# IamJerryXu/Multimodal-Diagnosis-HAM-Spine

Hardware: AMD Instinct MI355X
Metric: training images/sec, ResNet50+BERT-base 224px bs32 (higher is better)
Workload: dtype bf16; 1 GPU; C2: ResNet50 + BERT-base(L=128) + cross-attention FusionModule + MLP head, 224x224, batch 32 per GPU, CE(label_smoothing=0.02), fused AdamW, train-mode BatchNorm and dropout; per_gpu_batch=32, global_batch=32, seq_len=128, params=134897991, parallelism=dp1

## Files before the change

include/hamspine.h:

```cpp
#ifndef HAMSPINE_H
#define HAMSPINE_H

#include <stdint.h>

#ifdef __cplusplus
extern "C" {
#endif

typedef int hs_status;
enum { HS_OK = 0, HS_ERR_ARG = 1, HS_ERR_HIP = 2, HS_ERR_UNSUPPORTED = 3 };
enum { HS_F32 = 0, HS_BF16 = 1 };

const char* hs_last_error(void);
int hs_version(void);
int hs_device_ok(void);


enum {
    HS_A_KC = 0,
    HS_A_RC = 1,
    HS_A_CONV = 2,
    HS_A_DGRAD = 3
};
enum {
// ... 381 lines not shown
                            int32_t order, float grid_eps, float one_minus_eps, float margin, void* ws, int64_t ws_bytes,
                            void* stream);
int64_t hs_kan_refit_ws_bytes(int64_t B, int32_t in_f, int32_t out_f, int32_t grid_size, int32_t order, int32_t y_mode);
hs_status hs_kan_refit(const float* x, const float* grid_new, const float* grid_old, const float* y, const float* spline_w,
                       const float* scaler, float* out, int64_t B, int32_t in_f, int32_t out_f, int32_t grid_size, int32_t order,
                       void* ws, int64_t ws_bytes, void* stream);
hs_status hs_moe_gate_fwd(const float* clean, const float* raw_noise, const float* noise, int32_t B, int32_t E, int32_t k, int32_t noisy,
                          float noise_eps, uint64_t seed, float coef, float* gates, float* p, int32_t* top, float* z,
                          float* sigma, float* loadrow, float* loss, float* d_imp, float* d_load, void* stream);
hs_status hs_moe_gate_bwd(const float* clean, const float* raw_noise, const float* p, const int32_t* top, const float* z,
                          const float* sigma, const float* dgates, const float* g_loss, const float* d_imp,
                          const float* d_load, int32_t B, int32_t E, int32_t k, int32_t noisy, float* d_clean, float* d_raw,
                          void* stream);
hs_status hs_moe_combine_fwd(const float* gates, const float* const* outs, float* y, int32_t B, int32_t E, int32_t O,
                             void* stream);
hs_status hs_moe_combine_bwd(const float* gates, const float* const* outs, const float* dy, float* const* douts,
                             float* dgates, int32_t B, int32_t E, int32_t O, void* stream);

int32_t hs_pointwise_stat_rows(int64_t M, int32_t N, int32_t K);
hs_status hs_pointwise_fwd(const void* x, int64_t M, int32_t K, int32_t ldx, const void* w, int32_t N, void* y, int32_t ldy,
                           float* stats, void* stream);

hs_status hs_moe_dispatch_index(const float* gates, int32_t B, int32_t E, int32_t* idx, int32_t* count, void* stream);
hs_status hs_rows_gather(const float* src, const int32_t* idx, float* dst, int32_t n, int32_t D, void* stream);
hs_status hs_rows_scatter_add(float* dst, const int32_t* idx, const float* scale, int32_t ld_scale, int32_t col, const float* src,
                              int32_t n, int32_t D, void* stream);
hs_status hs_rows_scatter_add_bwd(const float* dy, const int32_t* idx, const float* gates, int32_t E, int32_t col, const float* src,
                                  float* dsrc, float* dgates, int32_t n, int32_t D, void* stream);


typedef struct hs_attn_desc {
    int32_t dtype;
    int32_t B, H, Lq, Lk, hd;
    int64_t q_bs, k_bs, v_bs, o_bs;
    int32_t q_ld, k_ld, v_ld, o_ld;
    float scale;
    float dropout_p;
    uint64_t seed;
    const int64_t* key_mask;
} hs_attn_desc;
hs_status hs_attention_query(const hs_attn_desc* d, int64_t* saved_bytes, int64_t* ws_bytes);
hs_status hs_attention_fwd(const hs_attn_desc* d, const void* q, const void* k, const void* v, void* o, void* saved,
                           int64_t saved_bytes, void* ws, int64_t ws_bytes, void* stream);
hs_status hs_attention_bwd(const hs_attn_desc* d, const void* q, const void* k, const void* v, const void* d_o, void* dq,
                           void* dk, void* dv, void* saved, int64_t saved_bytes, void* ws, int64_t ws_bytes,
                           void* stream);

void hs_set_overlap(int32_t on);
hs_status hs_grad_milestones(int32_t n, const void* const* grad_ptrs, void* const* events);
int32_t hs_measure_build(void);
void hs_set_wgrad_nt(int32_t on);
void hs_set_bert_wgrad_chunks(int32_t on);
void hs_set_pack_xcd_spread(int32_t on);
int64_t hs_gemm_k_cols_queued(void);

typedef struct hs_conv_bn {
    int32_t Cin, Cout, R, stride, pad;
    const float* w;
    const float* gamma;
    const float* beta;
    float* running_mean;
    float* running_var;
    float* dw;
    float* dgamma;
    float* dbeta;
} hs_conv_bn;

typedef struct hs_resblock_desc {
    int32_t dtype;
    int32_t N, H, W;
    int32_t training;
    float eps, momentum;
    int32_t n_main;
    hs_conv_bn main[3];
    int32_t has_ds;
    hs_conv_bn ds;
    int32_t inference;
} hs_resblock_desc;
hs_status hs_resblock_query(const hs_resblock_desc* d, int64_t* saved_bytes, int64_t* ws_bytes);
hs_status hs_resblock_fwd(const hs_resblock_desc* d, const void* x, void* y, void* saved, int64_t saved_bytes, void* ws,
                          int64_t ws_bytes, void* stream);
hs_status hs_resblock_bwd(const hs_resblock_desc* d, const void* x, const void* y, const void* dy, void* dx, void* saved,
                          int64_t saved_bytes, void* ws, int64_t ws_bytes, void* stream);

typedef struct hs_stem_desc {
    int32_t dtype;
    int32_t N, H, W;
    int32_t training;
    float eps, momentum;
    hs_conv_bn cb;
    int32_t inference;
} hs_stem_desc;
hs_status hs_stem_query(const hs_stem_desc* d, int64_t* saved_bytes, int64_t* ws_bytes);
hs_status hs_stem_fwd(const hs_stem_desc* d, const float* image, void* y, void* saved, int64_t saved_bytes, void* ws,
                      int64_t ws_bytes, void* stream);
hs_status hs_stem_bwd(const hs_stem_desc* d, const void* y, const void* dy, void* saved, int64_t saved_bytes, void* ws,
                      int64_t ws_bytes, void* stream);

typedef struct hs_linear {
    int32_t in_f, out_f;
    const float* w;
    const float* b;
    float* dw;
    float* db;
} hs_linear;
typedef struct hs_norm {
// ... 147 lines not shown
```

multimodal-diagnosis-ham-spine_amd/hamspine/csrc/gemm.hip:

```cpp
#include <atomic>
#include <mutex>
#include <unordered_set>
#include <vector>
#include <stdarg.h>
#include <math.h>
#include <map>
#include <tuple>
#include "gemm_launch.h"
#include "gemm_p8.h"
#include "hs_internal.h"
#include "hs_switch.h"

namespace hs {

static thread_local char g_err[512] = "";
void set_error(const char* fmt, ...) {
    va_list ap;
    va_start(ap, fmt);
    vsnprintf(g_err, sizeof(g_err), fmt, ap);
    va_end(ap);
}
const char* last_error() { return g_err; }

bool lds_attr_needed(const void* fn) {
// ... 22 lines not shown
        r.a = g_prof_pool.back().first;
        r.b = g_prof_pool.back().second;
        g_prof_pool.pop_back();
    } else if (hipEventCreate(&r.a) != hipSuccess || hipEventCreate(&r.b) != hipSuccess) {
        return false;
    }
    r.flops = flops;
    r.cls = cls;
    (void)hipEventRecord(r.a, s);
    return true;
}
static void prof_end(hipStream_t s, ProfRec& r) {
    (void)hipEventRecord(r.b, s);
    std::lock_guard<std::mutex> lk(g_prof_mu);
    g_prof.push_back(r);
}

__global__ void null_kernel() {}

static constexpr int kTicketPool = 16384;
static unsigned* ticket_pool(hipStream_t s) {
    static std::mutex mu;
    static std::map<std::pair<int, hipStream_t>, unsigned*> pools;
    int dev = 0;
    if (hipGetDevice(&dev) != hipSuccess) return nullptr;
    std::lock_guard<std::mutex> lk(mu);
    auto it = pools.find({dev, s});
    if (it != pools.end()) return it->second;
    unsigned* p = nullptr;
    if (hipMalloc(&p, kTicketPool * sizeof(unsigned)) != hipSuccess) return nullptr;
    if (hipMemsetAsync(p, 0, kTicketPool * sizeof(unsigned), s) != hipSuccess) return nullptr;
    pools[{dev, s}] = p;
    return p;
}

static int g_dbg_cfg = -1, g_dbg_ablate = 0;
static unsigned long long* g_dbg_stamps = nullptr;

static int combo_of(int ak, int bk) {
    if (ak == HS_A_KC && bk == HS_B_KC) return 0;
    if (ak == HS_A_KC && bk == HS_B_RC) return 1;
    if (ak == HS_A_RC && bk == HS_B_RC) return 2;
    if (ak == HS_A_CONV && bk == HS_B_KC) return 3;
    if (ak == HS_A_DGRAD && bk == HS_B_WDGRAD) return 4;
    if (ak == HS_A_RC && bk == HS_B_CONV) return 5;
    return -1;
}

static bool aligned16(const void* p) { return (((uintptr_t)p) & 15) == 0; }

static bool batch_is_one(const hs_gemm_params* p) { return p->batch <= 1; }
static int p8_cfg(const hs_gemm_params* p) {
    if (p->M % 256 == 0 && p->N % 256 == 0 && (long long)(p->M / 256) * (p->N / 256) >= 128) return CFG_P8_256;
    return -1;
}
static int auto_cfg(const hs_gemm_params* p, bool vec) {
    const long long z = (long long)(p->batch > 0 ? p->batch : 1) * (p->split_k > 1 ? p->split_k : 1);
    const long long t12864 = (long long)ceil_div(p->M, 128) * ceil_div(p->N, 64) * z;
    const long long t128 = (long long)ceil_div(p->M, 128) * ceil_div(p->N, 128) * z;
    if (p->dtype == HS_BF16) {
        const bool plain = (p->a_kind == HS_A_KC || p->a_kind == HS_A_RC) && (p->b_kind == HS_B_KC || p->b_kind == HS_B_RC);
        if (plain && batch_is_one(p)) {
            if (p->a_kind == HS_A_KC && p->split_k <= 1 && p->N >= 2048 && p->K <= 1024 && p->M >= 2048 && p->K % 32 == 0) return CFG_128x128x32;
            if (p->a_kind == HS_A_KC && p->b_kind == HS_B_KC && p->split_k <= 1 && p->K >= 2048 && t12864 >= 256) return CFG_128x64;
        }
        return t12864 >= 1536 ? CFG_128x64 : CFG_64x64;
    }
    return (vec && t128 >= 200) ? CFG_128x128 : CFG_64x64;
}
static bool conv3_plan(const hs_gemm_params* p, int* rows, int* tpi, int* fm) {
    if (!sw::conv3() || g_dbg_cfg >= 0) return false;
    const hs_conv_geom& g = p->g;
    if (p->dtype != HS_BF16 || p->a_kind != HS_A_CONV || p->b_kind != HS_B_KC || p->split_k > 1 || p->batch > 1) return false;
    if (g.R != 3 || g.S != 3 || g.stride != 1 || g.pad != 1 || g.P != g.H || g.Q != g.W || g.C % 64 != 0 || p->N % 64 != 0) return false;
    if (g.row_pitch != g.W * g.C || g.img_pitch != g.H * g.W * g.C || g.qstep != g.C || g.no_bounds) return false;
    if (p->bias || p->colscale || p->act != HS_ACT_NONE || p->residual || p->D_preact || p->mul_mode != HS_MUL_NONE || p->dropout_p > 0.f ||
        p->accumulate || p->seg_rows > 0 || p->alpha != 1.f || p->out_dtype != HS_BF16 || p->rowsum_a || p->bnb_partials)
        return false;
    if (p->ldd % 8 != 0 || (((uintptr_t)p->D) & 15) != 0 || p->ldb != 9 * g.C || p->K != 9 * g.C || p->N != g.K) return false;
    if (g.W > 112 || g.W < 1) return false;
    const int rmax = std::min(g.H, 112 / g.W);
    const int t = ceil_div(g.H, rmax), r = ceil_div(g.H, t);
    const int tp = r * g.W;
    if (tp < 32 || (r + 2) * (g.W + 2) > 256) return false;
    *rows = r;
    *tpi = t;
    *fm = tp > 64 ? 7 : 4;
    return true;
}
int gemm_stat_rows(const hs_gemm_params* p) {
    if (!p || p->dtype != HS_BF16 || p->split_k > 1 || p->batch > 1) return 0;
    {
        int r, t, fm;
        if (conv3_plan(p, &r, &t, &fm)) return p->g.N * t;
    }
    int cfg = (p->a_kind == HS_A_CONV && p->b_kind == HS_B_KC && p->g.C % 64 != 0) ? CFG_STEM : auto_cfg(p, true);
    if (g_dbg_cfg >= 0 && g_dbg_cfg <= CFG_64x64 && cfg != CFG_STEM) cfg = g_dbg_cfg;
    if (g_dbg_cfg >= CFG_256x128 && g_dbg_cfg <= CFG_256x128x32 && !(p->a_kind == HS_A_CONV || p->a_kind == HS_A_DGRAD || p->b_kind == HS_B_CONV)) cfg = g_dbg_cfg;
    return ceil_div(p->M, cfg == CFG_64x64 ? 64 : (cfg == CFG_256x128 || cfg == CFG_256x128x32) ? 256 : 128);
}

static bool bn_finish_variant(int cfg, int combo) {
    return (combo == 0 && (cfg == CFG_64x64 || cfg == CFG_128x64)) || (combo == 3 && (cfg == CFG_64x64 || cfg == CFG_128x64 || cfg == CFG_STEM || cfg == CFG_C3));
}

struct Prepared {
// ... 540 lines not shown
    if (g_group_immediate_hook) HS_PROPAGATE(g_group_immediate_hook(g_group_immediate_ctx));
    return gemm_impl(p, s);
}
bool gemm_group_takes_k_cols() { return g_dbg_cfg < 0 && !g_dbg_stamps; }
static std::atomic<long long> g_k_cols_queued{0};
int gemm_group_add(GemmGroup* g, const hs_gemm_params* p, hipStream_t s, const int* k_cols) {
    HS_REQUIRE(!k_cols || (g && p && p->a_kind == HS_A_KC && p->b_kind == HS_B_KC), "gemm_group_add: k_cols needs an open group and K-contiguous operands");
    if (!g) return launch_ungrouped(p, s);
    Prepared q;
    const bool big = p->a_kind == HS_A_KC && p->b_kind == HS_B_KC;
    const bool p8w = sw::p8_wgrad();
    const bool want_p8 = big && p8w && p->dtype == HS_BF16 && p->M % 256 == 0 && p->N % 256 == 0 && p->K % 64 == 0 && p->K >= 2048 &&
                         (p->batch <= 1) && p->split_k <= 1 && g_dbg_cfg < 0 && (g->items.empty() || g->combo != 0 || g->cfg == CFG_P8_256);
    HS_PROPAGATE(gemm_prepare(p, s, q, big ? (want_p8 ? CFG_P8_256 : CFG_256x128) : -1));
    if (want_p8 && !(p8_epilogue_supported(q.a) && !q.a.colstats && !q.a.bnb_partials && (long long)p->M * p->lda * 2 < 0x7fffff00ll &&
                     (long long)p->N * p->ldb * 2 < 0x7fffff00ll))
        HS_PROPAGATE(gemm_prepare(p, s, q, CFG_256x128));
    const bool ok = big ? (q.bf16 && (q.cfg == CFG_256x128 || q.cfg == CFG_P8_256) && q.combo == 0 && q.batch == 1 && q.split == 1 && !q.a.stamps && !q.a.colstats)
                        : (q.bf16 && q.cfg == CFG_64x64 && (q.combo == 2 || q.combo == 5) && q.batch == 1 && !q.a.stamps &&
                           (q.split == 1 || q.a.tickets != nullptr) && !q.a.colstats &&
                           (!q.a.rowsum[0] || (q.combo == 2 && q.split == 1)));
    HS_REQUIRE(!k_cols || ok, "gemm_group_add: a problem with chunk-compacted K columns cannot be queued (gemm_group_takes_k_cols)");
    if (!ok) return launch_ungrouped(p, s);
    const long long ngroups = q.split > 1 ? (q.split + kSplitGroup - 1) / kSplitGroup : 0;
    const long long need = q.split > 1 ? (long long)q.a.tiles_m * q.a.tiles_n * (1 + (ngroups > 1 ? ngroups : 0)) : 0;
    if (!g->items.empty() && (g->combo != q.combo || (big && g->cfg != q.cfg) || (int)g->items.size() >= kGroupMax || g->ticket_off + need > kTicketPool)) {
        if (g_group_immediate_hook) HS_PROPAGATE(g_group_immediate_hook(g_group_immediate_ctx));
        HS_PROPAGATE(gemm_group_flush(g, s));
    }
    if (need > kTicketPool) return launch_ungrouped(p, s);
    q.a.k_cols = k_cols;
    if (k_cols) g_k_cols_queued.fetch_add(1, std::memory_order_relaxed);
    g->combo = q.combo;
    if (big) {
        g->cfg = q.cfg;
        g->rs = g->rs || q.a.rowsum[0] != nullptr;
    }
    if (q.split > 1) q.a.tickets += g->ticket_off;
    g->ticket_off += (int)need;
    g->first.push_back(g->total);
    g->total += (int)(q.grid.x * q.grid.z);
    g->items.push_back(q.a);
    g->flops += q.flops;
    const double R2 = q.conv ? (double)p->g.R * p->g.S : 1.0, st2 = q.conv ? (double)p->g.stride * p->g.stride : 1.0;
    g->bytes += 2.0 * ((double)p->M * p->K + (double)p->N * p->K / R2 * st2) + 4.0 * (double)p->M * p->N;
    return HS_OK;
}

}

extern "C" {
void hs_gemm_debug_stamps(void* device_buffer) { hs::g_dbg_stamps = (unsigned long long*)device_buffer; }
void hs_set_pack_xcd_spread(int32_t on) { hs::sw::set_pack_xcd_spread(on); }
int64_t hs_gemm_k_cols_queued(void) { return hs::g_k_cols_queued.load(std::memory_order_relaxed); }
void hs_gemm_debug(int32_t cfg_override, int32_t ablate) {
    hs::g_dbg_cfg = cfg_override;
    hs::g_dbg_ablate = ablate;
}
void hs_prof_enable(int32_t on) {
    std::lock_guard<std::mutex> lk(hs::g_prof_mu);
    hs::g_prof_on = on != 0;
}
hs_status hs_prof_collect(double* flops, double* ms, int64_t* launches) {
    HS_CHECK_HIP(hipDeviceSynchronize());
    std::lock_guard<std::mutex> lk(hs::g_prof_mu);
    for (int i = 0; i < 4; ++i) {
        flops[i] = 0;
        ms[i] = 0;
        launches[i] = 0;
    }
    for (auto& r : hs::g_prof) {
        float t = 0.f;
        if (hipEventElapsedTime(&t, r.a, r.b) == hipSuccess) {
            flops[r.cls] += r.flops;
            ms[r.cls] += t;
            launches[r.cls] += 1;
        }
        hs::g_prof_pool.emplace_back(r.a, r.b);
    }
    hs::g_prof.clear();
    return HS_OK;
}
hs_status hs_prof_calibrate(void* stream, int32_t n, float* avg_us) {
    HS_REQUIRE(n > 0 && avg_us, "hs_prof_calibrate: bad argument");
    hipStream_t s = (hipStream_t)stream;
    std::vector<std::pair<hipEvent_t, hipEvent_t>> ev(n);
    for (auto& e : ev) {
        HS_CHECK_HIP(hipEventCreate(&e.first));
        HS_CHECK_HIP(hipEventCreate(&e.second));
    }
    for (auto& e : ev) {
        HS_CHECK_HIP(hipEventRecord(e.first, s));
        hipLaunchKernelGGL(hs::null_kernel, dim3(1), dim3(64), 0, s);
        HS_CHECK_HIP(hipEventRecord(e.second, s));
    }
    HS_CHECK_HIP(hipStreamSynchronize(s));
    double tot = 0;
    for (auto& e : ev) {
        float t = 0.f;
        HS_CHECK_HIP(hipEventElapsedTime(&t, e.first, e.second));
        tot += t;
        (void)hipEventDestroy(e.first);
        (void)hipEventDestroy(e.second);
    }
    *avg_us = (float)(tot / n * 1e3);
    return HS_OK;
// ... 50 lines not shown
```

multimodal-diagnosis-ham-spine_amd/hamspine/csrc/gemm_bf16_p8.hip:

```cpp
#include "gemm_launch.h"
#include "gemm_p8.h"
namespace hs {
__global__ __launch_bounds__(512) void gemm_bf16_p8_256_diag_kernel(const GemmArgs a) {
    gemm_bf16_p8_body<256, 256, 2, 4, false, true, true>(a, blockIdx.x);
}
template <typename K>
static int launch_p8(K kernel, int lds, int threads, const GemmArgs& a, dim3 grid, hipStream_t s) {
    if (lds_attr_needed((const void*)kernel)) HS_CHECK_HIP(hipFuncSetAttribute((const void*)kernel, hipFuncAttributeMaxDynamicSharedMemorySize, lds));
    hipLaunchKernelGGL(kernel, grid, dim3(threads), lds, s, a);
    HS_LAUNCH_CHECK();
    return HS_OK;
}
int launch_bf16_p8_grouped(const GemmArgs* list, const int* first_wg, int n, int total_wgs, bool rs, hipStream_t s) {
    constexpr int lds = 128 * 1024;
    if (rs) {
        auto kernel = gemm_bf16_p8_grouped_kernel<true>;
        if (lds_attr_needed((const void*)kernel)) HS_CHECK_HIP(hipFuncSetAttribute((const void*)kernel, hipFuncAttributeMaxDynamicSharedMemorySize, lds));
        hipLaunchKernelGGL(kernel, dim3(total_wgs), dim3(512), lds, s, list, first_wg, n);
    } else {
        auto kernel = gemm_bf16_p8_grouped_kernel<false>;
        if (lds_attr_needed((const void*)kernel)) HS_CHECK_HIP(hipFuncSetAttribute((const void*)kernel, hipFuncAttributeMaxDynamicSharedMemorySize, lds));
        hipLaunchKernelGGL(kernel, dim3(total_wgs), dim3(512), lds, s, list, first_wg, n);
    }
    HS_LAUNCH_CHECK();
    return HS_OK;
}
int launch_bf16_p8(int cfg, const GemmArgs& a, dim3 grid, hipStream_t s) {
    const bool rs = a.rowsum[0] != nullptr;
    switch (cfg) {
        case CFG_P8_256:
            if (a.stamps && !rs) return launch_p8(gemm_bf16_p8_256_diag_kernel, 128 * 1024, 512, a, grid, s);
            return rs ? launch_p8(gemm_bf16_p8_256_kernel<true>, 128 * 1024, 512, a, grid, s)
                      : launch_p8(gemm_bf16_p8_256_kernel<false>, 128 * 1024, 512, a, grid, s);
        case CFG_P8_256x128:
            return rs ? launch_p8(gemm_bf16_p8_256x128_kernel<true>, 96 * 1024, 512, a, grid, s)
                      : launch_p8(gemm_bf16_p8_256x128_kernel<false>, 96 * 1024, 512, a, grid, s);
        case CFG_P8_128:
            if (!rs) return launch_p8(gemm_bf16_p8_128_kernel<false>, 64 * 1024, 256, a, grid, s);
    }
    set_error("launch_bf16_p8: bad cfg %d (rowsum %d)", cfg, (int)rs);
    return HS_ERR_ARG;
}
}
```

multimodal-diagnosis-ham-spine_amd/hamspine/csrc/gemm_p8.h:

```cpp
#pragma once
#include "gemm_core.h"

namespace hs {

template <int N>
__device__ __forceinline__ void wait_vmcnt() {
    asm volatile("s_waitcnt vmcnt(%0)" ::"n"(N) : "memory");
}

template <int BM, int BN, int WGM, int WGN, bool RS, bool STAG, bool DIAG = false, int TAG = 0>
__device__ __forceinline__ void gemm_bf16_p8_body(const GemmArgs& a, const int bx) {
    typedef bf16_t T;
    constexpr int BK = 64, NW = WGM * WGN;
    constexpr int WM = BM / WGM, WN = BN / WGN;
    constexpr int QM = WM / 2, QN = WN / 2;
    constexpr int FMQ = QM / 16, FNQ = QN / 16;
    constexpr int FM = 2 * FMQ, FN = 2 * FNQ;
    constexpr int A_SLOT = (BM / 2) * BK * 2, B_SLOT = (BN / 2) * BK * 2;
    constexpr int BUF = 2 * A_SLOT + 2 * B_SLOT;
    constexpr int NA = A_SLOT / 1024 / NW, NB = B_SLOT / 1024 / NW;
    static_assert(QM % 16 == 0 && QN % 16 == 0 && NA >= 1 && NB >= 1 && A_SLOT % (1024 * NW) == 0 && B_SLOT % (1024 * NW) == 0, "tile / wave shape");
    static_assert(3 * NA + 3 * NB <= 63, "vmcnt field");
    extern __shared__ __attribute__((aligned(16))) char smem[];
    typedef __attribute__((address_space(3))) char lds_char;

    const int tid = threadIdx.x, lane = tid & 63;
    const int wave = __builtin_amdgcn_readfirstlane(tid >> 6);
    const int wm = wave / WGN, wn = wave % WGN;
    const int g = lane >> 4, l15 = lane & 15;
    int tm, tn;
    int tiles_m = a.tiles_m;
    if (a.m_rows && a.pack_spread) {
        tiles_m = min(tiles_m, max(0, (__builtin_amdgcn_readfirstlane(a.m_rows[0]) + BM - 1) / BM));
        if (bx >= tiles_m * a.tiles_n) return;
    }
    tile_from_block(a, tm, tn, bx, tiles_m);
    const int m0 = tm * BM, n0 = tn * BN;
    if (a.m_rows && m0 >= __builtin_amdgcn_readfirstlane(a.m_rows[0])) return;
    int ntiles = a.K / BK;
    if (a.k_cols) ntiles = max(1, min(ntiles, (__builtin_amdgcn_readfirstlane(a.k_cols[0]) + BK - 1) / BK));

    const __amdgpu_buffer_rsrc_t rsA = make_rsrc(a.A, (unsigned)min(a.a_bytes, 0x7fffff00ull));
    const __amdgpu_buffer_rsrc_t rsB = make_rsrc(a.B, (unsigned)min(a.b_bytes, 0x7fffff00ull));

    unsigned offA[2][NA], offB[2][NB];
#pragma unroll
    for (int q = 0; q < 2; ++q) {
#pragma unroll
        for (int i = 0; i < NA; ++i) {
            const int r = 8 * (wave * NA + i) + (lane >> 3);
            const int row = m0 + (r / QM) * WM + q * QM + (r % QM);
            offA[q][i] = (unsigned)row * (unsigned)a.lda * 2u + (unsigned)(((lane & 7) ^ kc_swz<8>(r)) << 4);
        }
#pragma unroll
        for (int i = 0; i < NB; ++i) {
            const int r = 8 * (wave * NB + i) + (lane >> 3);
            const int col = n0 + (r / QN) * WN + q * QN + (r % QN);
            offB[q][i] = (unsigned)col * (unsigned)a.ldb * 2u + (unsigned)(((lane & 7) ^ kc_swz<8>(r)) << 4);
        }
    }
    auto dma_a = [&](int t, int q) {
        if (t >= ntiles) return;
        lds_char* dst = (lds_char*)smem + (t & 1) * BUF + q * A_SLOT + wave * (NA * 1024);
        const int koff = t * (BK * 2);
#pragma unroll
        for (int i = 0; i < NA; ++i)
            __builtin_amdgcn_raw_ptr_buffer_load_lds(rsA, (__attribute__((address_space(3))) void*)(dst + i * 1024), 16, offA[q][i], koff, 0, 0);
    };
    auto dma_b = [&](int t, int q) {
        if (t >= ntiles) return;
        lds_char* dst = (lds_char*)smem + (t & 1) * BUF + 2 * A_SLOT + q * B_SLOT + wave * (NB * 1024);
        const int koff = t * (BK * 2);
#pragma unroll
        for (int i = 0; i < NB; ++i)
            __builtin_amdgcn_raw_ptr_buffer_load_lds(rsB, (__attribute__((address_space(3))) void*)(dst + i * 1024), 16, offB[q][i], koff, 0, 0);
    };

    bf16x8 af[FMQ][2], bq[2][FNQ][2];
    auto read_a = [&](int buf, int q) {
        const char* s = smem + buf * BUF + q * A_SLOT;
#pragma unroll
        for (int i = 0; i < FMQ; ++i)
#pragma unroll
            for (int ks = 0; ks < 2; ++ks) af[i][ks] = *(const bf16x8*)(s + kc_off_bf16<BK>(wm * QM + i * 16 + l15, ks * 4 + g));
    };
    auto read_b = [&](int buf, auto qc) {
        constexpr int q = decltype(qc)::value;
        const char* s = smem + buf * BUF + 2 * A_SLOT + q * B_SLOT;
#pragma unroll
        for (int j = 0; j < FNQ; ++j)
#pragma unroll
            for (int ks = 0; ks < 2; ++ks) bq[q][j][ks] = *(const bf16x8*)(s + kc_off_bf16<BK>(wn * QN + j * 16 + l15, ks * 4 + g));
    };

    constexpr int NDR = (WM + 63) / 64;
    int drow_v[NDR];
#pragma unroll
    for (int j = 0; j < NDR; ++j) drow_v[j] = 0;
    const bool have_drow = a.drop_rows != nullptr && a.drop_thresh != 0;
    if (have_drow) {
#pragma unroll
        for (int j = 0; j < NDR; ++j) drow_v[j] = ((const HS_GLOBAL int*)a.drop_rows)[min(m0 + wm * WM + j * 64 + lane, a.M - 1)];
    }
    f32x4 acc[FM][FN];
#pragma unroll
    for (int i = 0; i < FM; ++i)
#pragma unroll
        for (int j = 0; j < FN; ++j) acc[i][j] = f32x4{0.f, 0.f, 0.f, 0.f};
    f32x4 accb[RS ? FM : 1];
    bool do_rowsum = false;
    if constexpr (RS) {
        do_rowsum = a.rowsum[0] != nullptr && tn == 0 && wn == 0;
#pragma unroll
        for (int i = 0; i < FM; ++i) accb[i] = f32x4{0.f, 0.f, 0.f, 0.f};
    }
    auto mma = [&](auto qmc, auto qnc, bool with_rowsum) {
        constexpr int qm = decltype(qmc)::value, qn = decltype(qnc)::value;
        __builtin_amdgcn_s_setprio(1);
#pragma unroll
        for (int ks = 0; ks < 2; ++ks)
#pragma unroll
            for (int i = 0; i < FMQ; ++i)
#pragma unroll
                for (int j = 0; j < FNQ; ++j)
                    acc[qm * FMQ + i][qn * FNQ + j] =
                        __builtin_amdgcn_mfma_f32_16x16x32_bf16(bq[qn][j][ks], af[i][ks], acc[qm * FMQ + i][qn * FNQ + j], 0, 0, 0);
        if constexpr (RS) {
            if (with_rowsum && do_rowsum) {
                const s16x4 o4 = {0x3f80, 0x3f80, 0x3f80, 0x3f80};
                const bf16x8 ones = __builtin_bit_cast(bf16x8, __builtin_shufflevector(o4, o4, 0, 1, 2, 3, 4, 5, 6, 7));
#pragma unroll
                for (int ks = 0; ks < 2; ++ks)
#pragma unroll
                    for (int i = 0; i < FMQ; ++i)
                        accb[qm * FMQ + i] = __builtin_amdgcn_mfma_f32_16x16x32_bf16(ones, af[i][ks], accb[qm * FMQ + i], 0, 0, 0);
            }
        }
        __builtin_amdgcn_s_setprio(0);
    };
    auto fence_r = [&](auto nc, bool drain) {
        constexpr int N = decltype(nc)::value;
        if (drain) wait_vmcnt<0>();
        else if constexpr (N >= 0) wait_vmcnt<(N >= 0 ? N : 0)>();
        asm volatile("s_waitcnt lgkmcnt(0)" ::: "memory");
        __builtin_amdgcn_sched_barrier(0);
        __builtin_amdgcn_s_barrier();
        __builtin_amdgcn_sched_barrier(0);
    };
    auto fence_m = [&]() {
        __builtin_amdgcn_sched_barrier(0);
        __builtin_amdgcn_s_barrier();
        __builtin_amdgcn_sched_barrier(0);
    };
    using W_P0 = std::integral_constant<int, 2 * NA + 3 * NB>;
    using W_P1 = std::integral_constant<int, 3 * NA + 2 * NB>;
    using W_P2 = std::integral_constant<int, 3 * NA + 2 * NB>;
    using W_NONE = std::integral_constant<int, -1>;
    using I0 = std::integral_constant<int, 0>;
    using I1 = std::integral_constant<int, 1>;

    dma_a(0, 0); dma_b(0, 0); dma_b(0, 1); dma_a(0, 1);
    dma_a(1, 0); dma_b(1, 0); dma_b(1, 1);
    if (ntiles >= 2) wait_vmcnt<W_P0::value>();
    else wait_vmcnt<0>();
    __builtin_amdgcn_sched_barrier(0);
    __builtin_amdgcn_s_barrier();
    __builtin_amdgcn_sched_barrier(0);
    if constexpr (STAG) {
        if (wave >= NW / 2) {
            __builtin_amdgcn_s_barrier();
            __builtin_amdgcn_sched_barrier(0);
        }
    }

    unsigned long long stamp[DIAG ? 17 : 1];
    int nst = 0;
    auto STAMP = [&](int t) {
        if constexpr (DIAG) {
            if (t == ntiles / 2 && nst < 17) {
                __builtin_amdgcn_sched_barrier(0);
                stamp[nst++] = __builtin_readcyclecounter();
                __builtin_amdgcn_sched_barrier(0);
            }
        }
    };
    for (int t = 0; t < ntiles; ++t) {
        const int buf = t & 1;
        const bool tail = t + 2 >= ntiles;
        STAMP(t);
        read_a(buf, 0);
        read_b(buf, I0{});
        dma_a(t + 1, 1);
        if constexpr (DIAG) { asm volatile("s_waitcnt lgkmcnt(0)" ::: "memory"); STAMP(t); }
        fence_r(W_P1{}, tail);
        STAMP(t);
        mma(I0{}, I0{}, true);
        STAMP(t);
        fence_m();
        STAMP(t);
        read_b(buf, I1{});
        dma_a(t + 2, 0);
        if constexpr (DIAG) { asm volatile("s_waitcnt lgkmcnt(0)" ::: "memory"); STAMP(t); }
        fence_r(W_P2{}, tail);
        STAMP(t);
        mma(I0{}, I1{}, false);
        STAMP(t);
        fence_m();
        STAMP(t);
        read_a(buf, 1);
        dma_b(t + 2, 0);
        if constexpr (DIAG) { asm volatile("s_waitcnt lgkmcnt(0)" ::: "memory"); STAMP(t); }
        fence_r(W_NONE{}, false);
        STAMP(t);
        mma(I1{}, I1{}, true);
        STAMP(t);
        fence_m();
        STAMP(t);
        dma_b(t + 2, 1);
        fence_r(W_P0{}, tail);
        STAMP(t);
        mma(I1{}, I0{}, false);
        STAMP(t);
        fence_m();
    }
    if constexpr (DIAG) {
        if (a.stamps && lane == 0 && (wave == 0 || wave == NW / 2)) {
            unsigned long long* o = a.stamps + ((long long)bx * 2 + (wave ? 1 : 0)) * 20;
#pragma unroll
            for (int i = 0; i < 17; ++i) o[i] = stamp[i];
            o[17] = (unsigned long long)nst;
        }
    }
    if constexpr (STAG) {
        if (wave < NW / 2) __builtin_amdgcn_s_barrier();
    }
    wait_vmcnt<0>();

    const unsigned epi = epi_flags(a);
    if constexpr (RS) {
        if (do_rowsum && g == 0) {
#pragma unroll
            for (int i = 0; i < FM; ++i) {
                const int m = m0 + wm * WM + i * 16 + l15;
                const int seg = a.seg_rows > 0 ? m / a.seg_rows : 0;
                a.rowsum[seg][m - seg * (a.seg_rows > 0 ? a.seg_rows : 0)] = accb[i][0];
            }
        }
    }
    const unsigned key = epi & ~EPI_VEC16;
#define HS_EPI_CASE(F)                                                                                                        \
    case (F):                                                                                                                 \
        static_for<0, FM>([&](auto ic) {                                                                                      \
            constexpr int i = decltype(ic)::value;                                                                            \
            const int md1[1] = {have_drow ? __shfl(drow_v[(i * 16) / 64], (i * 16 + l15) & 63, 64) : -1};                         \
            run_epilogue<T, (F), true, 1, FN, 16, WN>(a, epi, *reinterpret_cast<f32x4(*)[1][FN]>(&acc[i]), m0 + wm * WM + i * 16, n0, 0, \
                                                      wn, l15, g, 0, 0, md1);                                                \
        });                                                                                                                   \
        break
    switch (key) {
        HS_EPI_CASE(EPI_VEC);
        HS_EPI_CASE(EPI_VEC | EPI_BIAS);
        HS_EPI_CASE(EPI_VEC | EPI_BIAS | EPI_GELU | EPI_PREACT);
        HS_EPI_CASE(EPI_VEC | EPI_BIAS | EPI_RES_POST);
        HS_EPI_CASE(EPI_VEC | EPI_BIAS | EPI_DROP | EPI_RES_POST);
        HS_EPI_CASE(EPI_VEC | EPI_MUL_GELU);
        HS_EPI_CASE(EPI_VEC | EPI_RES_POST);
        HS_EPI_CASE(EPI_VEC | EPI_OUT_F32);
        HS_EPI_CASE(EPI_VEC | EPI_OUT_F32 | EPI_SEG);
        default: break;
    }
#undef HS_EPI_CASE
}

inline bool p8_epilogue_supported(const GemmArgs& a) {
    unsigned f = 0;
    if (a.bias) f |= EPI_BIAS;
    if (a.colscale) f |= EPI_COLSCALE;
    if (a.mul_mode == HS_MUL_GELU_GRAD) f |= EPI_MUL_GELU;
    else if (a.mul_mode != HS_MUL_NONE) f |= EPI_MUL_RELU;
    if (a.seg_rows > 0) f |= EPI_SEG;
    if (a.D_preact) f |= EPI_PREACT;
    if (a.residual) f |= a.res_pre_act ? EPI_RES_PRE : EPI_RES_POST;
    if (a.act == HS_ACT_RELU) f |= EPI_RELU;
    else if (a.act == HS_ACT_GELU) f |= EPI_GELU;
    if (a.drop_thresh) f |= EPI_DROP;
    if (a.out_f32) f |= EPI_OUT_F32;
    if (a.accumulate) f |= EPI_ACCUM;
    if (a.vec_store) f |= EPI_VEC;
    if (a.parity) f |= EPI_PARITY;
    if (a.epi_generic || a.alpha != 1.f || a.res_gather) return false;
    if (!(f & EPI_OUT_F32) && !a.vec16) return false;
    switch (f) {
        case EPI_VEC: case EPI_VEC | EPI_BIAS: case EPI_VEC | EPI_BIAS | EPI_GELU | EPI_PREACT: case EPI_VEC | EPI_BIAS | EPI_RES_POST:
        case EPI_VEC | EPI_BIAS | EPI_DROP | EPI_RES_POST: case EPI_VEC | EPI_MUL_GELU: case EPI_VEC | EPI_RES_POST:
        case EPI_VEC | EPI_OUT_F32: case EPI_VEC | EPI_OUT_F32 | EPI_SEG:
            return true;
    }
    return false;
}

template <bool RS>
__global__ __launch_bounds__(512) void gemm_bf16_p8_256_kernel(const GemmArgs a) {
    gemm_bf16_p8_body<256, 256, 2, 4, RS, true>(a, blockIdx.x);
}
__global__ __launch_bounds__(512) void gemm_bf16_p8_256_diag_kernel(const GemmArgs a);
template <bool RS>
__global__ __launch_bounds__(512) void gemm_bf16_p8_grouped_kernel(const GemmArgs* __restrict__ list, const int* __restrict__ first_wg, int n) {
    const int bid = blockIdx.x, lane = threadIdx.x & 63;
    const int lo = lane < n ? first_wg[lane] : 0x7fffffff;
    const int p = __builtin_amdgcn_readfirstlane(__popcll(__ballot(lo <= bid)) - 1);
    const int local = bid - __builtin_amdgcn_readfirstlane(first_wg[p]);
    gemm_bf16_p8_body<256, 256, 2, 4, RS, true, false, 1>(list[p], local);
}
template <bool RS>
__global__ __launch_bounds__(512) void gemm_bf16_p8_256x128_kernel(const GemmArgs a) {
    gemm_bf16_p8_body<256, 128, 4, 2, RS, true>(a, blockIdx.x);
}
template <bool RS>
__global__ __launch_bounds__(256) void gemm_bf16_p8_128_kernel(const GemmArgs a) {
    gemm_bf16_p8_body<128, 128, 2, 2, RS, false>(a, blockIdx.x);
}

}
```

multimodal-diagnosis-ham-spine_amd/hamspine/csrc/hs_switch.h:

```cpp
#pragma once
#include <atomic>
#include <stdlib.h>

namespace hs {
namespace sw {

inline long long off_if_0(const char* e, long long d) { return (e && e[0] == '0') ? 0 : d; }
inline long long on_if_1(const char* e, long long d) { return (e && e[0] == '1') ? 1 : d; }
inline long long int_any(const char* e, long long d) { return e ? atoi(e) : d; }
inline long long int_mask15(const char* e, long long d) { return e ? (atoi(e) & 15) : d; }
inline long long int_1to8(const char* e, long long d) { const long long v = e ? atoi(e) : d; return v >= 1 && v <= 8 ? v : d; }
inline long long int_positive(const char* e, long long d) { const long long v = e ? atoll(e) : 0; return v > 0 ? v : d; }

#define HS_SWITCHES(X) \
   \
  X(p8,                 "HAMSPINE_P8",                  off_if_0,     1,   once,     -, "every GEMM on the generic body, none on the phase-pipelined one") \
  X(p8_wgrad,           "HAMSPINE_P8_WGRAD",            off_if_0,     1,   once,     -, "grouped deep-K weight gradients keep the generic 256x128 tiles") \
  X(conv3,              "HAMSPINE_CONV3",               off_if_0,     1,   once,     -, "3x3 stride-1 convolutions on the generic implicit GEMM, not the halo-patch kernel") \
  X(parity_dgrad,       "HAMSPINE_PARITY_DGRAD",        off_if_0,     1,   once,     -, "stride-2 data gradients keep the natural row order") \
  X(pack_xcd_spread,    "HAMSPINE_PACK_XCD_SPREAD",     off_if_0,     1,   settable, hs_set_pack_xcd_spread, "packed-row launches do not deal their live tiles over all XCDs") \
  X(persistent,         "HAMSPINE_PERSISTENT",          on_if_1,      0,   once,     -, "persistent GEMM launches (measured: no gain)") \
  X(epi_hist,           "HAMSPINE_EPI_HIST",            on_if_1,      0,   once,     -, "measurement: count the epilogue feature sets of the launches, print at exit") \
  X(group_debug,        "HAMSPINE_GROUP_DEBUG",         on_if_1,      0,   once,     -, "measurement: report every upload of a grouped launch's problem table") \
  X(split_units,        "HAMSPINE_SPLIT_UNITS",         int_positive, 512, once,     -, "measurement: the number of workgroups split-K aims at") \
  X(split_max,          "HAMSPINE_SPLIT_MAX",           int_positive, 64,  once,     -, "measurement: the largest split-K factor") \
   \
  X(fused_attention,    "HAMSPINE_FUSED_ATTENTION",     off_if_0,     1,   once,     -, "the unfused attention path") \
   \
  X(overlap,            "HAMSPINE_OVERLAP",             on_if_1,      0,   settable, hs_set_overlap, "a composite's weight gradients run on a side stream beside its data-gradient chain") \
  X(wgrad_nt,           "HAMSPINE_WGRAD_NT",            off_if_0,     1,   settable, hs_set_wgrad_nt, "BertLayer weight gradients from the row-major operands (tn); no packed rows then") \
  X(bert_wgrad_chunks,  "HAMSPINE_BERT_WGRAD_CHUNKS",   off_if_0,     1,   settable, hs_set_bert_wgrad_chunks, "packed text tower: weight gradients walk every padded column") \
  X(grouped_bert_wgrad, "HAMSPINE_GROUPED_BERT_WGRAD",  off_if_0,     1,   once,     -, "every weight-gradient GEMM of a BertLayer on its own") \
  X(wgrad_layers,       "HAMSPINE_WGRAD_LAYERS",        int_1to8,     2,   once,     -, "BERT layers whose weight gradients share one grouped grid (1: flush per layer)") \
  X(dgrad_nt,           "HAMSPINE_DGRAD_NT",            off_if_0,     1,   once,     -, "BERT data gradients read the row-contiguous weights") \
  X(defer_transposes,   "HAMSPINE_DEFER_TRANSPOSES",    off_if_0,     1,   once,     -, "one launch per dY^T where the gradient appears") \
  X(fused_bias_grad,    "HAMSPINE_FUSED_BIAS_GRAD",     off_if_0,     1,   once,     -, "bias gradients by separate column-sum passes") \
  X(fused_ln_bwd,       "HAMSPINE_FUSED_LN_BWD",        off_if_0,     1,   once,     -, "separate LayerNorm-backward / dropout / column-sum passes") \
  X(grouped_wgrad,      "HAMSPINE_GROUPED_WGRAD",       off_if_0,     1,   once,     -, "the image tower backward launches every weight gradient on its own") \
  X(staged_wgrad,       "HAMSPINE_STAGED_WGRAD",        off_if_0,     1,   once,     -, "with gradient milestones, the grouped weight gradients still run only at the end") \
  X(fused_bn_stats,     "HAMSPINE_FUSED_BN_STATS",      off_if_0,     1,   once,     -, "BatchNorm makes its own statistics pass") \
  X(bn_finish,          "HAMSPINE_BN_FINISH",           off_if_0,     1,   once,     -, "BatchNorm finishes its statistics in its own launch") \
  X(fused_bn_bwd,       "HAMSPINE_FUSED_BN_BWD",        off_if_0,     1,   once,     -, "BatchNorm backward makes its own partial-sum pass") \
  X(bnb_finish,         "HAMSPINE_BNB_FINISH",          on_if_1,      0,   once,     -, "the data-gradient GEMM also finishes the BatchNorm-backward sums (measured: no gain)") \
  X(bn_mask_from_x,     "HAMSPINE_BN_MASK_FROM_X",      on_if_1,      0,   once,     -, "inner-stage BatchNorm backward recomputes the ReLU mask from the convolution output (measured neutral)") \
  X(pw_stream,          "HAMSPINE_PW_STREAM",           on_if_1,      0,   once,     -, "1x1 convolutions of a training step through the streaming kernel (measured: a wash)") \
  X(xblock_bn,          "HAMSPINE_XBLOCK_BN",           int_any,      1,   per_call, -, "0: no BatchNorm sums across the block boundary; 2: on every eligible block, whatever its size") \
  X(ds_compact,         "HAMSPINE_DS_COMPACT",          off_if_0,     1,   per_call, -, "bf16 downsample data gradients keep the full-size parity-ordered route") \
  X(img_lean,           "HAMSPINE_IMG_LEAN",            int_mask15,   13,  per_call, -, "bit mask of the bf16 image tower's four lean passes (0: the separate launches)")
#define HS_SWITCHES_MEASURE(X) \
  X(knockout,           "HAMSPINE_KNOCKOUT",            int_any,      0,   once,     -, "bit mask of launch classes left OUT of the step (results are then garbage)")

#define HS_SW_once(id, name, rule, d) \
    inline long long id() { static const long long v = rule(getenv(name), d); return v; }
#define HS_SW_per_call(id, name, rule, d) \
    inline long long id() { return rule(getenv(name), d); }
#define HS_SW_settable(id, name, rule, d)                                                                   \
    inline std::atomic<int>& id##_cell() { static std::atomic<int> v{-1}; return v; }                        \
    inline void set_##id(int on) { id##_cell().store(on ? 1 : 0, std::memory_order_relaxed); }               \
    inline long long id() {                                                                                  \
        int v = id##_cell().load(std::memory_order_relaxed);                                                 \
        if (v < 0) {                                                                                         \
            const int env = (int)rule(getenv(name), d);                                                      \
            if (id##_cell().compare_exchange_strong(v, env, std::memory_order_relaxed)) v = env;             \
        }                                                                                                    \
        return v;                                                                                            \
    }
#define HS_SW_DEFINE(id, name, rule, d, latch, setter, doc) HS_SW_##latch(id, name, rule, d)

HS_SWITCHES(HS_SW_DEFINE)
#ifdef HS_MEASURE
HS_SWITCHES_MEASURE(HS_SW_DEFINE)
// ... 7 lines not shown
```

Before: 3330 images/s.

## Prefetch p8 GEMM LDS fragments one phase ahead and route mid-size deep-K GEMMs to p8_128

```diff
diff --git a/include/hamspine.h b/include/hamspine.h
--- a/include/hamspine.h
+++ b/include/hamspine.h
@@ -457,6 +457,7 @@
 void hs_set_wgrad_nt(int32_t on);
 void hs_set_bert_wgrad_chunks(int32_t on);
 void hs_set_pack_xcd_spread(int32_t on);
+void hs_set_p8_ahead(int32_t on);
 int64_t hs_gemm_k_cols_queued(void);
 
 typedef struct hs_conv_bn {
diff --git a/multimodal-diagnosis-ham-spine_amd/hamspine/csrc/gemm.hip b/multimodal-diagnosis-ham-spine_amd/hamspine/csrc/gemm.hip
--- a/multimodal-diagnosis-ham-spine_amd/hamspine/csrc/gemm.hip
+++ b/multimodal-diagnosis-ham-spine_amd/hamspine/csrc/gemm.hip
@@ -98,6 +98,10 @@
 static bool batch_is_one(const hs_gemm_params* p) { return p->batch <= 1; }
 static int p8_cfg(const hs_gemm_params* p) {
     if (p->M % 256 == 0 && p->N % 256 == 0 && (long long)(p->M / 256) * (p->N / 256) >= 128) return CFG_P8_256;
+    {
+        const long long t128 = (long long)(p->M / 128) * (p->N / 128);
+        if (p->K >= 2304 && p->M >= 2048 && p->M % 128 == 0 && p->N % 128 == 0 && t128 >= 192 && t128 <= 256) return CFG_P8_128;
+    }
     return -1;
 }
 static int auto_cfg(const hs_gemm_params* p, bool vec) {
@@ -744,6 +748,7 @@
 extern "C" {
 void hs_gemm_debug_stamps(void* device_buffer) { hs::g_dbg_stamps = (unsigned long long*)device_buffer; }
 void hs_set_pack_xcd_spread(int32_t on) { hs::sw::set_pack_xcd_spread(on); }
+void hs_set_p8_ahead(int32_t on) { hs::sw::set_p8_ahead(on); }
 int64_t hs_gemm_k_cols_queued(void) { return hs::g_k_cols_queued.load(std::memory_order_relaxed); }
 void hs_gemm_debug(int32_t cfg_override, int32_t ablate) {
     hs::g_dbg_cfg = cfg_override;
diff --git a/multimodal-diagnosis-ham-spine_amd/hamspine/csrc/gemm_bf16_p8.hip b/multimodal-diagnosis-ham-spine_amd/hamspine/csrc/gemm_bf16_p8.hip
--- a/multimodal-diagnosis-ham-spine_amd/hamspine/csrc/gemm_bf16_p8.hip
+++ b/multimodal-diagnosis-ham-spine_amd/hamspine/csrc/gemm_bf16_p8.hip
@@ -1,8 +1,10 @@
 #include "gemm_launch.h"
 #include "gemm_p8.h"
+#include "hs_switch.h"
 namespace hs {
+template <bool AH>
 __global__ __launch_bounds__(512) void gemm_bf16_p8_256_diag_kernel(const GemmArgs a) {
-    gemm_bf16_p8_body<256, 256, 2, 4, false, true, true>(a, blockIdx.x);
+    gemm_bf16_p8_body<256, 256, 2, 4, false, true, AH, true>(a, blockIdx.x);
 }
 template <typename K>
 static int launch_p8(K kernel, int lds, int threads, const GemmArgs& a, dim3 grid, hipStream_t s) {
@@ -11,33 +13,41 @@
     HS_LAUNCH_CHECK();
     return HS_OK;
 }
-int launch_bf16_p8_grouped(const GemmArgs* list, const int* first_wg, int n, int total_wgs, bool rs, hipStream_t s) {
+template <typename K>
+static int launch_p8_grouped(K kernel, const GemmArgs* list, const int* first_wg, int n, int total_wgs, hipStream_t s) {
     constexpr int lds = 128 * 1024;
-    if (rs) {
-        auto kernel = gemm_bf16_p8_grouped_kernel<true>;
-        if (lds_attr_needed((const void*)kernel)) HS_CHECK_HIP(hipFuncSetAttribute((const void*)kernel, hipFuncAttributeMaxDynamicSharedMemorySize, lds));
-        hipLaunchKernelGGL(kernel, dim3(total_wgs), dim3(512), lds, s, list, first_wg, n);
-    } else {
-        auto kernel = gemm_bf16_p8_grouped_kernel<false>;
-        if (lds_attr_needed((const void*)kernel)) HS_CHECK_HIP(hipFuncSetAttribute((const void*)kernel, hipFuncAttributeMaxDynamicSharedMemorySize, lds));
-        hipLaunchKernelGGL(kernel, dim3(total_wgs), dim3(512), lds, s, list, first_wg, n);
-    }
+    if (lds_attr_needed((const void*)kernel)) HS_CHECK_HIP(hipFuncSetAttribute((const void*)kernel, hipFuncAttributeMaxDynamicSharedMemorySize, lds));
+    hipLaunchKernelGGL(kernel, dim3(total_wgs), dim3(512), lds, s, list, first_wg, n);
     HS_LAUNCH_CHECK();
     return HS_OK;
 }
+int launch_bf16_p8_grouped(const GemmArgs* list, const int* first_wg, int n, int total_wgs, bool rs, hipStream_t s) {
+    const bool ah = sw::p8_ahead() != 0;
+    if (rs) return ah ? launch_p8_grouped(gemm_bf16_p8_grouped_kernel<true, true>, list, first_wg, n, total_wgs, s)
+                      : launch_p8_grouped(gemm_bf16_p8_grouped_kernel<true, false>, list, first_wg, n, total_wgs, s);
+    return ah ? launch_p8_grouped(gemm_bf16_p8_grouped_kernel<false, true>, list, first_wg, n, total_wgs, s)
+              : launch_p8_grouped(gemm_bf16_p8_grouped_kernel<false, false>, list, first_wg, n, total_wgs, s);
+}
 int launch_bf16_p8(int cfg, const GemmArgs& a, dim3 grid, hipStream_t s) {
     const bool rs = a.rowsum[0] != nullptr;
+    const bool ah = sw::p8_ahead() != 0;
+#define HS_P8_PICK(kernel, lds, threads)                                                                  \
+    (rs ? (ah ? launch_p8(kernel<true, true>, lds, threads, a, grid, s) : launch_p8(kernel<true, false>, lds, threads, a, grid, s)) \
+        : (ah ? launch_p8(kernel<false, true>, lds, threads, a, grid, s) : launch_p8(kernel<false, false>, lds, threads, a, grid, s)))
     switch (cfg) {
         case CFG_P8_256:
-            if (a.stamps && !rs) return launch_p8(gemm_bf16_p8_256_diag_kernel, 128 * 1024, 512, a, grid, s);
-            return rs ? launch_p8(gemm_bf16_p8_256_kernel<true>, 128 * 1024, 512, a, grid, s)
-                      : launch_p8(gemm_bf16_p8_256_kernel<false>, 128 * 1024, 512, a, grid, s);
+            if (a.stamps && !rs)
+                return ah ? launch_p8(gemm_bf16_p8_256_diag_kernel<true>, 128 * 1024, 512, a, grid, s)
+                          : launch_p8(gemm_bf16_p8_256_diag_kernel<false>, 128 * 1024, 512, a, grid, s);
+            return HS_P8_PICK(gemm_bf16_p8_256_kernel, 128 * 1024, 512);
         case CFG_P8_256x128:
-            return rs ? launch_p8(gemm_bf16_p8_256x128_kernel<true>, 96 * 1024, 512, a, grid, s)
-                      : launch_p8(gemm_bf16_p8_256x128_kernel<false>, 96 * 1024, 512, a, grid, s);
+            return HS_P8_PICK(gemm_bf16_p8_256x128_kernel, 96 * 1024, 512);
         case CFG_P8_128:
-            if (!rs) return launch_p8(gemm_bf16_p8_128_kernel<false>, 64 * 1024, 256, a, grid, s);
+            if (!rs)
+                return ah ? launch_p8(gemm_bf16_p8_128_kernel<false, true>, 64 * 1024, 256, a, grid, s)
+                          : launch_p8(gemm_bf16_p8_128_kernel<false, false>, 64 * 1024, 256, a, grid, s);
     }
+#undef HS_P8_PICK
     set_error("launch_bf16_p8: bad cfg %d (rowsum %d)", cfg, (int)rs);
     return HS_ERR_ARG;
 }
diff --git a/multimodal-diagnosis-ham-spine_amd/hamspine/csrc/gemm_p8.h b/multimodal-diagnosis-ham-spine_amd/hamspine/csrc/gemm_p8.h
--- a/multimodal-diagnosis-ham-spine_amd/hamspine/csrc/gemm_p8.h
+++ b/multimodal-diagnosis-ham-spine_amd/hamspine/csrc/gemm_p8.h
@@ -8,7 +8,7 @@
     asm volatile("s_waitcnt vmcnt(%0)" ::"n"(N) : "memory");
 }
 
-template <int BM, int BN, int WGM, int WGN, bool RS, bool STAG, bool DIAG = false, int TAG = 0>
+template <int BM, int BN, int WGM, int WGN, bool RS, bool STAG, bool AHEAD, bool DIAG = false, int TAG = 0>
 __device__ __forceinline__ void gemm_bf16_p8_body(const GemmArgs& a, const int bx) {
     typedef bf16_t T;
     constexpr int BK = 64, NW = WGM * WGN;
@@ -21,6 +21,7 @@
     constexpr int NA = A_SLOT / 1024 / NW, NB = B_SLOT / 1024 / NW;
     static_assert(QM % 16 == 0 && QN % 16 == 0 && NA >= 1 && NB >= 1 && A_SLOT % (1024 * NW) == 0 && B_SLOT % (1024 * NW) == 0, "tile / wave shape");
     static_assert(3 * NA + 3 * NB <= 63, "vmcnt field");
+    constexpr bool AF2 = AHEAD && (FM * FN * 4 + (RS ? FM * 4 : 0) + 4 * (2 * FMQ * 2 + 2 * FNQ * 2) + 30 <= 256);
     extern __shared__ __attribute__((aligned(16))) char smem[];
     typedef __attribute__((address_space(3))) char lds_char;
 
@@ -76,21 +77,22 @@
             __builtin_amdgcn_raw_ptr_buffer_load_lds(rsB, (__attribute__((address_space(3))) void*)(dst + i * 1024), 16, offB[q][i], koff, 0, 0);
     };
 
-    bf16x8 af[FMQ][2], bq[2][FNQ][2];
-    auto read_a = [&](int buf, int q) {
+    bf16x8 af[AF2 ? 2 : 1][FMQ][2], bq[2][FNQ][2];
+    auto read_a = [&](int buf, int q, auto setc) {
+        constexpr int set = decltype(setc)::value;
         const char* s = smem + buf * BUF + q * A_SLOT;
 #pragma unroll
         for (int i = 0; i < FMQ; ++i)
 #pragma unroll
-            for (int ks = 0; ks < 2; ++ks) af[i][ks] = *(const bf16x8*)(s + kc_off_bf16<BK>(wm * QM + i * 16 + l15, ks * 4 + g));
-    };
-    auto read_b = [&](int buf, auto qc) {
-        constexpr int q = decltype(qc)::value;
+            for (int ks = 0; ks < 2; ++ks) af[set][i][ks] = *(const bf16x8*)(s + kc_off_bf16<BK>(wm * QM + i * 16 + l15, ks * 4 + g));
+    };
+    auto read_b = [&](int buf, int q, auto setc) {
+        constexpr int set = decltype(setc)::value;
         const char* s = smem + buf * BUF + 2 * A_SLOT + q * B_SLOT;
 #pragma unroll
         for (int j = 0; j < FNQ; ++j)
 #pragma unroll
-            for (int ks = 0; ks < 2; ++ks) bq[q][j][ks] = *(const bf16x8*)(s + kc_off_bf16<BK>(wn * QN + j * 16 + l15, ks * 4 + g));
+            for (int ks = 0; ks < 2; ++ks) bq[set][j][ks] = *(const bf16x8*)(s + kc_off_bf16<BK>(wn * QN + j * 16 + l15, ks * 4 + g));
     };
 
     constexpr int NDR = (WM + 63) / 64;
@@ -114,8 +116,8 @@
 #pragma unroll
         for (int i = 0; i < FM; ++i) accb[i] = f32x4{0.f, 0.f, 0.f, 0.f};
     }
-    auto mma = [&](auto qmc, auto qnc, bool with_rowsum) {
-        constexpr int qm = decltype(qmc)::value, qn = decltype(qnc)::value;
+    auto mma = [&](auto qmc, auto qnc, auto asc, auto bsc, bool with_rowsum) {
+        constexpr int qm = decltype(qmc)::value, qn = decltype(qnc)::value, as = decltype(asc)::value, bs = decltype(bsc)::value;
         __builtin_amdgcn_s_setprio(1);
 #pragma unroll
         for (int ks = 0; ks < 2; ++ks)
@@ -124,7 +126,7 @@
 #pragma unroll
                 for (int j = 0; j < FNQ; ++j)
                     acc[qm * FMQ + i][qn * FNQ + j] =
-                        __builtin_amdgcn_mfma_f32_16x16x32_bf16(bq[qn][j][ks], af[i][ks], acc[qm * FMQ + i][qn * FNQ + j], 0, 0, 0);
+                        __builtin_amdgcn_mfma_f32_16x16x32_bf16(bq[bs][j][ks], af[as][i][ks], acc[qm * FMQ + i][qn * FNQ + j], 0, 0, 0);
         if constexpr (RS) {
             if (with_rowsum && do_rowsum) {
                 const s16x4 o4 = {0x3f80, 0x3f80, 0x3f80, 0x3f80};
@@ -133,21 +135,22 @@
                 for (int ks = 0; ks < 2; ++ks)
 #pragma unroll
                     for (int i = 0; i < FMQ; ++i)
-                        accb[qm * FMQ + i] = __builtin_amdgcn_mfma_f32_16x16x32_bf16(ones, af[i][ks], accb[qm * FMQ + i], 0, 0, 0);
+                        accb[qm * FMQ + i] = __builtin_amdgcn_mfma_f32_16x16x32_bf16(ones, af[as][i][ks], accb[qm * FMQ + i], 0, 0, 0);
             }
         }
         __builtin_amdgcn_s_setprio(0);
     };
-    auto fence_r = [&](auto nc, bool drain) {
+    auto fence_r = [&](auto nc, bool drain, auto lgkmc) {
         constexpr int N = decltype(nc)::value;
         if (drain) wait_vmcnt<0>();
         else if constexpr (N >= 0) wait_vmcnt<(N >= 0 ? N : 0)>();
-        asm volatile("s_waitcnt lgkmcnt(0)" ::: "memory");
+        if constexpr (decltype(lgkmc)::value != 0) asm volatile("s_waitcnt lgkmcnt(0)" ::: "memory");
         __builtin_amdgcn_sched_barrier(0);
         __builtin_amdgcn_s_barrier();
         __builtin_amdgcn_sched_barrier(0);
     };
     auto fence_m = [&]() {
+        if constexpr (AHEAD) asm volatile("s_waitcnt lgkmcnt(0)" ::: "memory");
         __builtin_amdgcn_sched_barrier(0);
         __builtin_amdgcn_s_barrier();
         __builtin_amdgcn_sched_barrier(0);
@@ -155,17 +158,27 @@
     using W_P0 = std::integral_constant<int, 2 * NA + 3 * NB>;
     using W_P1 = std::integral_constant<int, 3 * NA + 2 * NB>;
     using W_P2 = std::integral_constant<int, 3 * NA + 2 * NB>;
+    using W_AH = std::integral_constant<int, 2 * NA + 2 * NB>;
     using W_NONE = std::integral_constant<int, -1>;
+    using LGKM = std::integral_constant<int, 1>;
+    using LGKM_A = std::integral_constant<int, AF2 ? 0 : 1>;
+    using NO_LGKM = std::integral_constant<int, 0>;
     using I0 = std::integral_constant<int, 0>;
     using I1 = std::integral_constant<int, 1>;
 
     dma_a(0, 0); dma_b(0, 0); dma_b(0, 1); dma_a(0, 1);
     dma_a(1, 0); dma_b(1, 0); dma_b(1, 1);
-    if (ntiles >= 2) wait_vmcnt<W_P0::value>();
+    if (ntiles >= 2) wait_vmcnt<AHEAD ? W_AH::value : W_P0::value>();
     else wait_vmcnt<0>();
     __builtin_amdgcn_sched_barrier(0);
     __builtin_amdgcn_s_barrier();
     __builtin_amdgcn_sched_barrier(0);
+    if constexpr (AHEAD) {
+        if constexpr (AF2) read_a(0, 0, I0{});
+        read_b(0, 0, I0{});
+        asm volatile("s_waitcnt lgkmcnt(0)" ::: "memory");
+        __builtin_amdgcn_sched_barrier(0);
+    }
     if constexpr (STAG) {
         if (wave >= NW / 2) {
             __builtin_amdgcn_s_barrier();
@@ -184,44 +197,76 @@
             }
         }
     };
-    for (int t = 0; t < ntiles; ++t) {
-        const int buf = t & 1;
+    auto tile = [&](const int t, auto pc) __attribute__((always_inline)) {
+        constexpr int P0 = AHEAD ? decltype(pc)::value : 0;
+        using S0 = std::integral_constant<int, P0>;
+        using S1 = std::integral_constant<int, 1 - P0>;
+        using A1 = std::integral_constant<int, AF2 ? 1 : 0>;
+        const int buf = AHEAD ? P0 : (t & 1);
         const bool tail = t + 2 >= ntiles;
-        STAMP(t);
-        read_a(buf, 0);
-        read_b(buf, I0{});
+        const bool last = t + 1 >= ntiles;
+        STAMP(t);
+        if constexpr (AHEAD) {
+            if constexpr (!AF2) read_a(buf, 0, I0{});
+            read_b(buf, 1, S1{});
+        } else {
+            read_a(buf, 0, I0{});
+            read_b(buf, 0, S0{});
+        }
         dma_a(t + 1, 1);
-        if constexpr (DIAG) { asm volatile("s_waitcnt lgkmcnt(0)" ::: "memory"); STAMP(t); }
-        fence_r(W_P1{}, tail);
-        STAMP(t);
-        mma(I0{}, I0{}, true);
+        if constexpr (DIAG) { if constexpr (!AHEAD) asm volatile("s_waitcnt lgkmcnt(0)" ::: "memory"); STAMP(t); }
+        if constexpr (AHEAD) fence_r(W_AH{}, last, LGKM_A{});
+        else fence_r(W_P1{}, tail, LGKM{});
+        STAMP(t);
+        mma(I0{}, I0{}, I0{}, S0{}, true);
         STAMP(t);
         fence_m();
         STAMP(t);
-        read_b(buf, I1{});
+        if constexpr (AHEAD) {
+            if constexpr (AF2) read_a(buf, 1, I1{});
+        } else {
+            read_b(buf, 1, S1{});
+        }
         dma_a(t + 2, 0);
-        if constexpr (DIAG) { asm volatile("s_waitcnt lgkmcnt(0)" ::: "memory"); STAMP(t); }
-        fence_r(W_P2{}, tail);
-        STAMP(t);
-        mma(I0{}, I1{}, false);
+        if constexpr (DIAG) { if constexpr (!AHEAD) asm volatile("s_waitcnt lgkmcnt(0)" ::: "memory"); STAMP(t); }
+        if constexpr (AHEAD) fence_r(W_NONE{}, false, NO_LGKM{});
+        else fence_r(W_P2{}, tail, LGKM{});
+        STAMP(t);
+        mma(I0{}, I1{}, I0{}, S1{}, false);
         STAMP(t);
         fence_m();
         STAMP(t);
-        read_a(buf, 1);
+        if constexpr (!AF2) read_a(buf, 1, I0{});
         dma_b(t + 2, 0);
-        if constexpr (DIAG) { asm volatile("s_waitcnt lgkmcnt(0)" ::: "memory"); STAMP(t); }
-        fence_r(W_NONE{}, false);
-        STAMP(t);
-        mma(I1{}, I1{}, true);
+        if constexpr (DIAG) { if constexpr (!AHEAD) asm volatile("s_waitcnt lgkmcnt(0)" ::: "memory"); STAMP(t); }
+        if constexpr (AHEAD) fence_r(W_AH{}, tail, LGKM_A{});
+        else fence_r(W_NONE{}, false, LGKM{});
+        STAMP(t);
+        mma(I1{}, I1{}, A1{}, S1{}, true);
         STAMP(t);
         fence_m();
         STAMP(t);
+        if constexpr (AHEAD) {
+            if (!last) {
+                if constexpr (AF2) read_a(buf ^ 1, 0, I0{});
+                read_b(buf ^ 1, 0, S1{});
+            }
+        }
         dma_b(t + 2, 1);
-        fence_r(W_P0{}, tail);
-        STAMP(t);
-        mma(I1{}, I0{}, false);
+        if constexpr (AHEAD) fence_r(W_AH{}, tail, NO_LGKM{});
+        else fence_r(W_P0{}, tail, LGKM{});
+        STAMP(t);
+        mma(I1{}, I0{}, A1{}, S0{}, false);
         STAMP(t);
         fence_m();
+    };
+    if constexpr (AHEAD) {
+        for (int t = 0; t < ntiles; t += 2) {
+            tile(t, I0{});
+            if (t + 1 < ntiles) tile(t + 1, I1{});
+        }
+    } else {
+        for (int t = 0; t < ntiles; ++t) tile(t, I0{});
     }
     if constexpr (DIAG) {
         if (a.stamps && lane == 0 && (wave == 0 || wave == NW / 2)) {
@@ -299,26 +344,27 @@
     return false;
 }
 
-template <bool RS>
+template <bool RS, bool AH>
 __global__ __launch_bounds__(512) void gemm_bf16_p8_256_kernel(const GemmArgs a) {
-    gemm_bf16_p8_body<256, 256, 2, 4, RS, true>(a, blockIdx.x);
-}
+    gemm_bf16_p8_body<256, 256, 2, 4, RS, true, AH>(a, blockIdx.x);
+}
+template <bool AH>
 __global__ __launch_bounds__(512) void gemm_bf16_p8_256_diag_kernel(const GemmArgs a);
-template <bool RS>
+template <bool RS, bool AH>
 __global__ __launch_bounds__(512) void gemm_bf16_p8_grouped_kernel(const GemmArgs* __restrict__ list, const int* __restrict__ first_wg, int n) {
     const int bid = blockIdx.x, lane = threadIdx.x & 63;
     const int lo = lane < n ? first_wg[lane] : 0x7fffffff;
     const int p = __builtin_amdgcn_readfirstlane(__popcll(__ballot(lo <= bid)) - 1);
     const int local = bid - __builtin_amdgcn_readfirstlane(first_wg[p]);
-    gemm_bf16_p8_body<256, 256, 2, 4, RS, true, false, 1>(list[p], local);
-}
-template <bool RS>
+    gemm_bf16_p8_body<256, 256, 2, 4, RS, true, AH, false, 1>(list[p], local);
+}
+template <bool RS, bool AH>
 __global__ __launch_bounds__(512) void gemm_bf16_p8_256x128_kernel(const GemmArgs a) {
-    gemm_bf16_p8_body<256, 128, 4, 2, RS, true>(a, blockIdx.x);
-}
-template <bool RS>
+    gemm_bf16_p8_body<256, 128, 4, 2, RS, true, AH>(a, blockIdx.x);
+}
+template <bool RS, bool AH>
 __global__ __launch_bounds__(256) void gemm_bf16_p8_128_kernel(const GemmArgs a) {
-    gemm_bf16_p8_body<128, 128, 2, 2, RS, false>(a, blockIdx.x);
-}
-
-}
+    gemm_bf16_p8_body<128, 128, 2, 2, RS, false, AH>(a, blockIdx.x);
+}
+
+}
diff --git a/multimodal-diagnosis-ham-spine_amd/hamspine/csrc/hs_switch.h b/multimodal-diagnosis-ham-spine_amd/hamspine/csrc/hs_switch.h
--- a/multimodal-diagnosis-ham-spine_amd/hamspine/csrc/hs_switch.h
+++ b/multimodal-diagnosis-ham-spine_amd/hamspine/csrc/hs_switch.h
@@ -16,7 +16,8 @@
    \
   X(p8,                 "HAMSPINE_P8",                  off_if_0,     1,   once,     -, "every GEMM on the generic body, none on the phase-pipelined one") \
   X(p8_wgrad,           "HAMSPINE_P8_WGRAD",            off_if_0,     1,   once,     -, "grouped deep-K weight gradients keep the generic 256x128 tiles") \
-  X(conv3,              "HAMSPINE_CONV3",               off_if_0,     1,   once,     -, "3x3 stride-1 convolutions on the generic implicit GEMM, not the halo-patch kernel") \
+  X(p8_ahead,           "HAMSPINE_P8_AHEAD",            off_if_0,     1,   settable, hs_set_p8_ahead, "the phase-pipelined body reads each phase's fragments in that phase, not one phase ahead") \
+  X(conv3,              "HAMSPINE_CONV3",              off_if_0,     1,   once,     -, "3x3 stride-1 convolutions on the generic implicit GEMM, not the halo-patch kernel") \
   X(parity_dgrad,       "HAMSPINE_PARITY_DGRAD",        off_if_0,     1,   once,     -, "stride-2 data gradients keep the natural row order") \
   X(pack_xcd_spread,    "HAMSPINE_PACK_XCD_SPREAD",     off_if_0,     1,   settable, hs_set_pack_xcd_spread, "packed-row launches do not deal their live tiles over all XCDs") \
   X(persistent,         "HAMSPINE_PERSISTENT",          on_if_1,      0,   once,     -, "persistent GEMM launches (measured: no gain)") \
```

New measurement: 3346 images/s (median of 6 runs). No clear change (+0.5%).
